# mpriessner/MultiModalSpectralTransformer

Measured on NVIDIA B200. Metric: generated SMILES tokens/sec, higher is better.
Workload: dtype bf16

## Files before the change

### multimodalspectraltransformer_b200/csrc/engine.cu

```cuda
#include "engine.cuh"
#include "kernels_simt.cuh"
#include "kernels_tc.cuh"
#include "kernels_decode.cuh"
#include "kernels_ffn.cuh"
#include "kernels_attn5.cuh"
#include "kernels_compact.cuh"
#include "kernels_beam.cuh"
#include "kernels_smiles.cuh"

#include <algorithm>
#include <cstdlib>
#include <cstring>

namespace mmt {
thread_local std::string g_last_error;

static const char* kEmbedKeys[5] = {
    "linear_spec_embedding_1H.point_embedding_layer_1H.fc_H",
    "linear_spec_embedding_13C.point_embedding_layer_13C.fc_C",
    "linear_spec_embedding_HSQC.point_embedding_layer_HSQC.fc_HSQC",
    "linear_spec_embedding_COSY.point_embedding_layer_COSY.fc_COSY",
    "linear_spec_embedding_IR.linear_spec_embedding_IR"};
static const char* kEncNames[6] = {"encoder_1H", "encoder_13C", "encoder_HSQC", "encoder_COSY", "encoder_IR", "encoder_cross"};

static void prof_pre(mmt_engine* e, cudaStream_t s) {
    if (!e->profiling) return;
    cudaEvent_t a, b;
    cudaEventCreate(&a); cudaEventCreate(&b);
    cudaEventRecord(a, s);
    e->prof_open = {a, b};
}
static int check_launch(mmt_engine* e, const char* what, cudaStream_t s = nullptr, double work = 0.0) {
    e->launches++;
    cudaError_t err = cudaGetLastError();
    if (e->profiling && e->prof_open.first) {
        cudaEventRecord(e->prof_open.second, s);
        e->prof_records.push_back({what, e->prof_open.first, e->prof_open.second, work});
        e->prof_open = {nullptr, nullptr};
// ... 98 lines not shown
}

static int launch_ln(mmt_engine* e, LnParams& p, int ngroups, int maxM, cudaStream_t s) {
    if (maxM <= 0) return 0;
    dim3 grid((maxM + 7) / 8, ngroups);
    prof_pre(e, s);
    bias_res_layernorm<<<grid, 256, 0, s>>>(p);
    return check_launch(e, "bias_res_layernorm", s);
}

typedef CUresult (*PFN_tmapEncodeTiled)(CUtensorMap*, CUtensorMapDataType, cuuint32_t, void*, const cuuint64_t*, const cuuint64_t*,
                                        const cuuint32_t*, const cuuint32_t*, CUtensorMapInterleave, CUtensorMapSwizzle,
                                        CUtensorMapL2promotion, CUtensorMapFloatOOBfill);
static PFN_tmapEncodeTiled g_encode_tiled = nullptr;

static int tc_init(mmt_engine* e) {
    if (e->tc_ready) return 0;
    if (!g_encode_tiled) {
        void* fn = nullptr;
        cudaDriverEntryPointQueryResult qres;
        MMT_CUDA(cudaGetDriverEntryPoint("cuTensorMapEncodeTiled", &fn, cudaEnableDefault, &qres));
        if (!fn || qres != cudaDriverEntryPointSuccess) MMT_FAIL("cuTensorMapEncodeTiled not available from the driver");
        g_encode_tiled = (PFN_tmapEncodeTiled)fn;
    }
    const int max_smem = TC_MAX_STAGES * TC_STAGE_BYTES_WSPLIT + 1024;
    MMT_CUDA(cudaFuncSetAttribute(gemm_bf16_tc<TC_EPI_STORE>, cudaFuncAttributeMaxDynamicSharedMemorySize, max_smem));
    MMT_CUDA(cudaFuncSetAttribute(gemm_bf16_tc<TC_EPI_LN>, cudaFuncAttributeMaxDynamicSharedMemorySize, max_smem));
    MMT_CUDA(cudaFuncSetAttribute(attn_encoder_tc5, cudaFuncAttributeMaxDynamicSharedMemorySize, A5_SMEM_BYTES));
    MMT_CUDA(cudaFuncSetAttribute(ffn_fused_tc<TC_EPI_STORE, 1>, cudaFuncAttributeMaxDynamicSharedMemorySize, ff_smem_bytes<1>()));
    MMT_CUDA(cudaFuncSetAttribute(ffn_fused_tc<TC_EPI_LN, 1>, cudaFuncAttributeMaxDynamicSharedMemorySize, ff_smem_bytes<1>()));
    MMT_CUDA(cudaFuncSetAttribute(ffn_fused_tc<TC_EPI_STORE, 0>, cudaFuncAttributeMaxDynamicSharedMemorySize, ff_smem_bytes<0>()));
    MMT_CUDA(cudaFuncSetAttribute(ffn_fused_tc<TC_EPI_LN, 0>, cudaFuncAttributeMaxDynamicSharedMemorySize, ff_smem_bytes<0>()));
    MMT_CUDA(cudaFuncSetAttribute(ffn_fused_tc<TC_EPI_LN, 0, 1>, cudaFuncAttributeMaxDynamicSharedMemorySize, ff_smem_bytes<0, 1>()));
    e->tc_ready = true;
    return 0;
}

static int make_tmap(CUtensorMap* m, const __nv_bfloat16* ptr, int64_t rows, int64_t cols, int64_t ld, int box_rows = TC_BM) {
    if (((uintptr_t)ptr & 15) || (ld * 2) % 16) MMT_FAIL("tensor map: operand must be 16-byte aligned with a 16-byte multiple row pitch");
    cuuint64_t dims[2] = {(cuuint64_t)cols, (cuuint64_t)rows};
    cuuint64_t strides[1] = {(cuuint64_t)ld * 2};
    cuuint32_t box[2] = {(cuuint32_t)TC_BK, (cuuint32_t)box_rows};
    cuuint32_t estr[2] = {1, 1};
    CUresult r = g_encode_tiled(m, CU_TENSOR_MAP_DATA_TYPE_BFLOAT16, 2, (void*)ptr, dims, strides, box, estr, CU_TENSOR_MAP_INTERLEAVE_NONE,
                                CU_TENSOR_MAP_SWIZZLE_128B, CU_TENSOR_MAP_L2_PROMOTION_L2_256B, CU_TENSOR_MAP_FLOAT_OOB_FILL_NONE);
    if (r != CUDA_SUCCESS) MMT_FAIL("cuTensorMapEncodeTiled failed with CUresult " + std::to_string((int)r));
    return 0;
}

static TcGemmParams tc_params(int M, int N, int K) {
    TcGemmParams p;
    memset(&p, 0, sizeof(p));
    p.M = M; p.N = N; p.K = K; p.splits = 1; p.eps = 1e-5f;
    p.S_in = M > 0 ? M : 1; p.stride_b = 0; p.stride_s = 1; p.off = 0;
    return p;
}

static int sample_init(mmt_engine* e) {
    if (e->sample_ready) return 0;
    MMT_CUDA(cudaFuncSetAttribute(sample_tokens, cudaFuncAttributeMaxDynamicSharedMemorySize, (int)sample_smem_bytes(VOCAB_MAX)));
    e->sample_ready = true;
    return 0;
}

struct TcChain { const __nv_bfloat16 *W, *Wlo; const float* bias; float* out; int64_t ld; };
static int launch_tc(mmt_engine* e, TcGemmParams& p, const __nv_bfloat16* A, int64_t lda, const __nv_bfloat16* W, int epi, cudaStream_t s,
// ... 757 lines not shown
        p.bias = w.in_b; p.out_f32 = b.qkv; p.ld_f32 = e->use_kv_epilogue ? D : 3 * D;
        p.kv_append = e->use_kv_epilogue ? (e->kv_tok_major && H % 8 == 0 ? 2 : 1) : 0; p.kv_pool = reinterpret_cast<__nv_bfloat16*>(pool); p.block_table = b.block_table; p.pps = pps; p.step = step; p.kv_heads = H;
        MMT_TRY(launch_tc(e, p, b.x16, D, e->Wb(w.in_w), TC_EPI_STORE, s, e->dec_proj_single ? nullptr : e->Wlo(w.in_w), pdl_u));
    } else {
        GemmParams p = gemm_params(3 * D, D, 3 * D, 0);
        p.g[0].A = b.x; p.g[0].lda = D; p.g[0].W = w.in_w; p.g[0].bias = w.in_b; p.g[0].C = b.qkv; p.g[0].M = M;
        p.splits = 1; p.part_stride = Nw * D;
        MMT_TRY(launch_gemm(e, p, 1, M, s));
    }
    prof_pre(e, s);
    const unsigned sa_blocks = (unsigned)((Nw * (H / 4) + 7) / 8);
    if (bf16 && e->use_kv_epilogue && e->kv_tok_major && H % 8 == 0)
        launch_args(decode_self_attention_tm<8>, dim3((unsigned)((Nw * (H / 8) + 7) / 8)), dim3(256), 0, s, pdl_u, (const float*)b.qkv, (const __nv_bfloat16*)reinterpret_cast<__nv_bfloat16*>(pool), (const int*)b.block_table, pps, Nw, H, scale, step, b.att16);
    else if (bf16 && e->use_kv_epilogue) launch_args(decode_self_attention_g8<8, __nv_bfloat16, false>, dim3(sa_blocks), dim3(256), 0, s, pdl_u, (const float*)b.qkv, reinterpret_cast<__nv_bfloat16*>(pool), (const int*)b.block_table, pps, Nw, H, scale, step, (float*)nullptr, b.att16);
    else if (bf16) launch_args(decode_self_attention_g8<8, __nv_bfloat16>, dim3(sa_blocks), dim3(256), 0, s, pdl_u, (const float*)b.qkv, reinterpret_cast<__nv_bfloat16*>(pool), (const int*)b.block_table, pps, Nw, H, scale, step, (float*)nullptr, b.att16);
    else decode_self_attention_g8<8, float><<<sa_blocks, 256, 0, s>>>(b.qkv, reinterpret_cast<float*>(pool), b.block_table, pps, Nw, H, scale, step, b.att, b.att16);
    return check_launch(e, "decode_self_attention", s);
}

static int decode_cross_attention_layer(mmt_engine* e, const mmt_decode_args& a, const DecBuffers& b, const char* ckv, int64_t Nw, int Bmw,
                                        bool bf16, bool pdl_u, cudaStream_t s) {
    const int H = e->desc.n_heads, dh = D / H;
    const float scale = 1.0f / sqrtf((float)dh);
    if (dh != 8) MMT_FAIL("decoder head dim must be 8");
    const unsigned attn_blocks = (unsigned)((Nw * H + 7) / 8);
    prof_pre(e, s);
    if (bf16 && a.n_cand >= 8 && e->use_tc_attention)
        launch_args(decode_cross_attention_tc, dim3(H, Bmw), dim3(256), dx_smem_bytes(a.S), s, pdl_u, (const float*)b.qc, reinterpret_cast<const __nv_bfloat16*>(ckv), (int64_t)a.S, (const int*)b.nk, (const int*)b.row_start, (const float*)b.kbias_c, (int)a.n_cand, H, scale, (float*)nullptr, b.att16);
    else if (bf16) launch_args(decode_cross_attention<8, __nv_bfloat16>, dim3(attn_blocks), dim3(256), 0, s, pdl_u, (const float*)b.qc, reinterpret_cast<const __nv_bfloat16*>(ckv), (int64_t)a.S, (const int*)b.nk, (const int*)b.row_start, (const float*)b.kbias_c, (int)a.n_cand, Nw, H, scale, (float*)nullptr, b.att16);
    else decode_cross_attention<8, float><<<attn_blocks, 256, 0, s>>>(b.qc, reinterpret_cast<const float*>(ckv), a.S, b.nk, b.row_start, b.kbias_c, a.n_cand, Nw, H, scale, b.att, b.att16);
    return check_launch(e, "decode_cross_attention", s);
}

struct DecOps {
    mmt_engine* e; const DecBuffers& b; int64_t Nw; bool pdl_u; cudaStream_t s;
    int ln(const float* part, int splits, const float* bias, const float* gamma, const float* beta) const {
        LnParams q;
        memset(&q, 0, sizeof(q));
        q.splits = splits; q.part_stride = Nw * D; q.eps = 1e-5f;
        LnGroup& g = q.g[0];
        g.part = part; g.bias = bias; g.res = b.x; g.gamma = gamma; g.beta = beta; g.out = b.x; g.out_bf16 = b.x16; g.M = (int)Nw;
        g.S_in = (int)Nw; g.stride_b = 0; g.stride_s = 1; g.off = 0;
        return launch_ln(e, q, 1, (int)Nw, s);
    }
    int gemm(const float* A, int64_t lda, const float* W, const float* bias, float* C, int N, int K, int act, int splits) const {
        GemmParams p = gemm_params(N, K, N, act);
        p.g[0].A = A; p.g[0].lda = lda; p.g[0].W = W; p.g[0].bias = bias; p.g[0].C = C; p.g[0].M = (int)Nw;
        p.splits = splits; p.part_stride = Nw * D;
        return launch_gemm(e, p, 1, (int)Nw, s);
    }
    const __nv_bfloat16* plo(const float* w) const { return e->dec_proj_single ? nullptr : e->Wlo(w); }
    const __nv_bfloat16* dlo(const float* w) const { return e->dec_ffn_single ? nullptr : e->Wlo(w); }
    int tc(const __nv_bfloat16* A, int64_t lda, const float* W, const float* bias, float* C32, __nv_bfloat16* C16, int N, int K, int act, int splits) const {
        TcGemmParams p = tc_params((int)Nw, N, K);
        p.bias = bias; p.act = act; p.out_f32 = C32; p.ld_f32 = N; p.out_b16 = C16; p.ld_b16 = N;
        p.splits = splits; p.part_stride = Nw * D;
        return launch_tc(e, p, A, lda, e->Wb(W), TC_EPI_STORE, s, plo(W), pdl_u);
    }
    int tc_ln(const __nv_bfloat16* A, int64_t lda, const float* W, const float* bias, int K, const float* gamma, const float* beta,
              const TcChain* chain = nullptr) const {
        TcGemmParams p = tc_params((int)Nw, D, K);
        p.bias = bias; p.res = b.x; p.gamma = gamma; p.beta = beta;
        p.out_f32 = b.x; p.ld_f32 = D; p.out_b16 = b.x16; p.ld_b16 = D;
        return launch_tc(e, p, A, lda, e->Wb(W), TC_EPI_LN, s, plo(W), pdl_u, chain);
    }
};

static int decode_self_tail_layer(const DecOps& o, const LayerW& w, bool bf16) {
    const DecBuffers& b = o.b;
    if (bf16) {
        if (o.e->use_gemm_chain && o.Nw <= 24576) {
            const TcChain ch{o.e->Wb(w.ca_in_w), o.plo(w.ca_in_w), w.ca_in_b, b.qc, D};
            MMT_TRY(o.tc_ln(b.att16, D, w.out_w, w.out_b, D, w.n1_w, w.n1_b, &ch));
        } else {
            MMT_TRY(o.tc_ln(b.att16, D, w.out_w, w.out_b, D, w.n1_w, w.n1_b));
            MMT_TRY(o.tc(b.x16, D, w.ca_in_w, w.ca_in_b, b.qc, nullptr, D, D, 0, 1));
        }
    } else {
        MMT_TRY(o.gemm(b.att, D, w.out_w, nullptr, b.part, D, D, 0, 1));
        MMT_TRY(o.ln(b.part, 1, w.out_b, w.n1_w, w.n1_b));
        MMT_TRY(o.gemm(b.x, D, w.ca_in_w, w.ca_in_b, b.qc, D, D, 0, 1));
    }
    return 0;
}

static int decode_cross_tail_layer(const DecOps& o, const LayerW& w, int l, bool bf16, float* x2 = nullptr) {
    mmt_engine* e = o.e;
    const DecBuffers& b = o.b;
    const int M = (int)o.Nw, F = e->desc.d_ff;
    cudaStream_t s = o.s;
    auto keep_x2 = [&]() -> int {
        if (x2) MMT_CUDA(cudaMemcpyAsync(x2, b.x, (size_t)M * D * sizeof(float), cudaMemcpyDeviceToDevice, s));
        return 0;
    };
    if (bf16) {
        const bool ffn_pro = e->use_ffn_prologue && M >= 2048;
        if (!ffn_pro) { MMT_TRY(o.tc_ln(b.att16, D, w.ca_out_w, w.ca_out_b, D, w.n2_w, w.n2_b)); MMT_TRY(keep_x2()); }
        if (M >= 2048) {
            FfnParams f = ffn_params(M, F);
            f.b1 = w.l1_b; f.bias = w.l2_b; f.res = b.x; f.gamma = w.n3_w; f.beta = w.n3_b; f.out_f32 = b.x; f.out_b16 = b.x16;
            if (getenv("MMT_FFN_DEBUG")) {
                if (!e->ffn_dbg) { MMT_CUDA(cudaMallocManaged(&e->ffn_dbg, 4096 * 16 * sizeof(long long))); memset(e->ffn_dbg, 0, 4096 * 16 * sizeof(long long)); }
// ... 77 lines not shown
            if (cl_ffn) {
                MMT_TRY(tc_init(e));
                MMT_TRY(make_tmap(&q.tmW1, e->Wb(w.l1_w), d.d_ff, D, D));
                MMT_TRY(make_tmap(&q.tmW2, e->Wb(w.l2_w), D, d.d_ff, d.d_ff));
                q.b1 = w.l1_b; q.b2 = w.l2_b; q.n3_w = w.n3_w; q.n3_b = w.n3_b; q.x_out = b.x;
            }
            q.in_w = w.in_w; q.in_b = w.in_b; q.out_w = w.out_w; q.out_b = w.out_b; q.n1_w = w.n1_w; q.n1_b = w.n1_b;
            q.kv_pool = b.kv_pool + (size_t)l * b.pool_pages * 2 * PAGE_TOKENS * D * b.kv_esz; q.block_table = b.block_table; q.pps = pps;
            q.step = step;
            q.in_w16 = e->Wb(w.in_w); q.out_w16 = e->Wb(w.out_w); q.cq_w16 = e->Wb(w.ca_in_w); q.co_w16 = e->Wb(w.ca_out_w);
            q.cq_w = w.ca_in_w; q.cq_b = w.ca_in_b; q.co_w = w.ca_out_w; q.co_b = w.ca_out_b; q.n2_w = w.n2_w; q.n2_b = w.n2_b;
            q.ckv = b.cross_kv + (size_t)l * 2 * R * D * b.kv_esz; q.rows_total = a.S;
            q.nk = b.nk; q.row_start = b.row_start; q.kbias_c = b.kbias_c; q.n_cand = a.n_cand;
            q.x2 = b.x; q.x2_16 = bf16 ? b.x16 : nullptr; q.M = Nw; q.scale = scale; q.eps = 1e-5f;
            q.dbg = (e->da_dbg && l == 3) ? e->da_dbg : nullptr;
            prof_pre(e, s);
            const bool pdl_l = pdl && !(l == 0 && r.serial_first);
            if (cl_ffn) launch_kernel_cluster(decode_attn<8, __nv_bfloat16, true>, dim3(blocks), dim3(DA_THREADS), DA_SMEM_BYTES_CL, s, pdl_l, DA_CL, q);
            else if (bf16) launch_kernel(decode_attn<8, __nv_bfloat16>, dim3(blocks), dim3(DA_THREADS), DA_SMEM_BYTES, s, pdl_l, q);
            else launch_kernel(decode_attn<8, float>, dim3(blocks), dim3(DA_THREADS), DA_SMEM_BYTES, s, pdl_l, q);
            MMT_TRY(check_launch(e, "decode_attn", s));
            if (cl_ffn) continue;
            if (bf16) {
                FfnParams f = ffn_params(M, d.d_ff);
                f.b1 = w.l1_b; f.splits = ffn_splits; f.out_f32 = b.part; f.part_stride = Nw * D;
                f.dbg = (e->da_dbg && l == 3) ? e->da_dbg + 2048 * 16 : nullptr;
                MMT_TRY(launch_ffn(e, f, b.x16, D, e->Wb(w.l1_w), o.dlo(w.l1_w), e->Wb(w.l2_w), o.dlo(w.l2_w), TC_EPI_STORE, s, pdl));
            } else {
                MMT_TRY(o.gemm(b.x, D, w.l1_w, w.l1_b, b.h, d.d_ff, D, 1, 1));
                MMT_TRY(o.gemm(b.h, d.d_ff, w.l2_w, nullptr, b.part, D, d.d_ff, 0, ffn_splits));
            }
        }
    } else {
        prof_pre(e, s);
        if (r.trg) launch_args(decode_embed, dim3((unsigned)((Nw + 3) / 4)), dim3(128), 0, s, pdl_u, r.trg + n0, 0, 3, Nw, ldn, e->W("embed_trg.weight"), e->W("pe_trg.weight"), (int)d.vocab, step, b.x, b.x16);
        else launch_args(decode_embed, dim3((unsigned)((Nw + 3) / 4)), dim3(128), 0, s, pdl_u, (const int64_t*)(r.tokens + n0), 1, 3, Nw, ldn, e->W("embed_trg.weight"), e->W("pe_trg.weight"), (int)d.vocab, step, b.x, b.x16);
        MMT_TRY(check_launch(e, "decode_embed", s));

        for (int l = 0; l < d.n_dec_layers; ++l) {
            const LayerW& w = e->dec[l];
            char* pool = b.kv_pool + (size_t)l * b.pool_pages * 2 * PAGE_TOKENS * D * b.kv_esz;
            const char* ckv = b.cross_kv + (size_t)l * 2 * R * D * b.kv_esz;
            MMT_TRY(decode_self_attention_layer(e, w, b, pool, pps, Nw, bf16, pdl_u, s));
            MMT_TRY(decode_self_tail_layer(o, w, bf16));
            MMT_TRY(decode_cross_attention_layer(e, a, b, ckv, Nw, Bmw, bf16, pdl_u, s));
            MMT_TRY(decode_cross_tail_layer(o, w, l, bf16));
        }
    }
    SampleParams sp;
    memset(&sp, 0, sizeof(sp));
    sp.x = b.x; sp.W = e->W("fc_out.weight"); sp.b = e->W("fc_out.bias"); sp.V = d.vocab; sp.N = Nw; sp.ldn = ldn;
    sp.temperature = a.temperature; sp.mode = r.mode;
    int smc = a.rng_sm_count > 0 ? a.rng_sm_count : e->sm_count;
    int mts = a.rng_max_threads_per_sm > 0 ? a.rng_max_threads_per_sm : e->max_threads_per_sm;
    int64_t Nrng = r.per_memory_rng ? a.n_cand : (a.N_total > 0 ? a.N_total : N_total);
    sp.rng.seed = a.philox_seed; sp.rng.offset = a.philox_offset; sp.rng.numel = Nrng * d.vocab;
    sp.rng.threads = torch_rng_threads(sp.rng.numel, smc, mts);
    sp.rng_inc = torch_rng_increment(sp.rng.numel, smc, mts);
    sp.rng_dev = b.rng_state;
    sp.seq_index_base = a.seq_index_base + n0;
    if (r.per_memory_rng) { sp.rng_cand = a.n_cand; sp.rng_col_steps = a.max_len; }
    sp.tokens = r.tokens ? r.tokens + n0 : nullptr; sp.probs = r.probs ? r.probs + n0 : nullptr;
    sp.logits = r.logits ? r.logits + n0 * d.vocab : nullptr;
    sp.target = r.target ? r.target + n0 : nullptr; sp.target_prob = r.target_prob ? r.target_prob + n0 : nullptr;
    sp.ctl.step = b.ctl; sp.ctl.done_ctas = b.ctl + 1; sp.ctl.nonpad = (r.mode == 0) ? b.ctl + 8 : nullptr;
    sp.advance = 1;
    if (fused && ffn_splits > 0) {
        const LayerW& pw = e->dec[d.n_dec_layers - 1];
        sp.part = b.part; sp.splits = ffn_splits; sp.part_stride = Nw * D;
        sp.pbias = pw.l2_b; sp.pgamma = pw.n3_w; sp.pbeta = pw.n3_b; sp.eps = 1e-5f;
    }
    prof_pre(e, s);
    {
        sp.rows_per_warp = Nw >= 8192 ? SAMPLE_NR : 1;
        const int rpc = sp.part ? 2 : 8 * sp.rows_per_warp;
        const int64_t groups = (Nw + rpc - 1) / rpc;
        MMT_TRY(sample_init(e));
        launch_kernel(sample_tokens, dim3((unsigned)std::min<int64_t>(groups, (int64_t)e->sm_count * 4)), dim3(256), sample_smem_bytes(sp.V), s, pdl || pdl_u, sp);
// ... 346 lines not shown
}
int64_t mmt_weight_total(const mmt_model_desc* desc) { if (check_desc(desc)) return -1; return build_registry(*desc).total; }

int32_t mmt_create(const mmt_model_desc* desc, const float* h_weights, int64_t n_floats, int32_t device, mmt_engine** out) {
    if (!out) MMT_FAIL("null out");
    *out = nullptr;
    MMT_TRY(check_desc(desc));
    int ndev = 0;
    if (cudaGetDeviceCount(&ndev) != cudaSuccess || ndev == 0) MMT_FAIL("no CUDA device: this engine has no CPU fallback");
    if (device < 0 || device >= ndev) MMT_FAIL("bad device index");
    cudaDeviceProp prop;
    MMT_CUDA(cudaGetDeviceProperties(&prop, device));
    if (prop.major != 10) MMT_FAIL(std::string("device is sm_") + std::to_string(prop.major * 10 + prop.minor) + "; this library is built for sm_100a (B200) only");
    MMT_CUDA(cudaSetDevice(device));
    mmt_engine* e = new mmt_engine();
    e->desc = *desc; e->device = device; e->sm_count = prop.multiProcessorCount; e->max_threads_per_sm = prop.maxThreadsPerMultiProcessor; e->total_mem = prop.totalGlobalMem;
    e->reg = build_registry(*desc);
    if (getenv("MMT_NO_GRAPH")) e->use_graph = false;
    if (getenv("MMT_NO_PDL")) e->use_pdl = false;
    if (getenv("MMT_NO_GRAPH_CACHE")) e->use_graph_cache = false;
    if (const char* v = getenv("MMT_GRAPH_STEPS")) e->graph_steps = std::max(1, atoi(v));
    if (getenv("MMT_NO_ENC_STREAMS")) e->use_enc_streams = false;
    if (const char* v = getenv("MMT_DECODE_LANES")) e->decode_lanes = std::max(1, atoi(v));
    if (getenv("MMT_DENSE_ENCODER")) e->use_compact = false;
    if (getenv("MMT_NO_TC_ATTENTION")) e->use_tc_attention = false;
    if (getenv("MMT_TC5_ATTENTION")) e->use_tc5_attention = true;
    if (const char* v = getenv("MMT_FFN_SPLITS")) { int k = atoi(v); if (k == 1 || k == 2 || k == 4 || k == 8 || k == 16 || k == 32) e->ffn_splits_override = k; }
    if (getenv("MMT_TC_ATTENTION_FP32")) e->tc_attention_fp32 = true;
    if (const char* v = getenv("MMT_FUSED_DECODE_ROWS")) e->fused_decode_rows = atoi(v);
    if (getenv("MMT_DEC_FFN_TWO_TERM")) e->dec_ffn_single = false;
    if (getenv("MMT_DEC_PROJ_TWO_TERM")) e->dec_proj_single = false;
    if (const char* v = getenv("MMT_PDL_ROWS")) e->pdl_rows = atoi(v);
    if (getenv("MMT_NO_GEMM_CHAIN")) e->use_gemm_chain = false;
    if (getenv("MMT_NO_FFN_WIDE")) e->use_ffn_wide = false;
    if (getenv("MMT_NO_KV_EPILOGUE")) e->use_kv_epilogue = false;
    if (getenv("MMT_KV_HEAD_MAJOR")) e->kv_tok_major = false;
    if (getenv("MMT_CLUSTER_FFN")) e->use_cluster_ffn = true;
    if (getenv("MMT_NO_FFN_PROLOGUE")) e->use_ffn_prologue = false;
    if (getenv("MMT_ENC_FFN_SINGLE")) e->enc_ffn_single = true;
    if (const char* v = getenv("MMT_DECODE_LANES_LARGE")) e->decode_lanes_large = std::max(1, atoi(v));
    if (const char* v = getenv("MMT_MAX_WAVE_SEQS")) e->max_wave_seqs = std::max(1, atoi(v));
    if (n_floats != e->reg.total) { delete e; MMT_FAIL("weight blob has " + std::to_string(n_floats) + " floats, expected " + std::to_string(build_registry(*desc).total)); }
    auto fail = [&](const std::string& m) { mmt_destroy(e); g_last_error = m; return 1; };
    if (cudaMalloc(&e->w32, n_floats * sizeof(float)) != cudaSuccess) return fail("cudaMalloc weights failed");
    if (cudaMalloc(&e->w16, n_floats * sizeof(__nv_bfloat16)) != cudaSuccess) return fail("cudaMalloc bf16 weights failed");
    if (cudaMemcpy(e->w32, h_weights, n_floats * sizeof(float), cudaMemcpyHostToDevice) != cudaSuccess) return fail("weight H2D copy failed");
    if (cudaMalloc(&e->w16lo, n_floats * sizeof(__nv_bfloat16)) != cudaSuccess) return fail("cudaMalloc bf16 weights (low term) failed");
    f32_to_bf16_split<<<(unsigned)((n_floats + 255) / 256), 256>>>(e->w32, n_floats, e->w16, e->w16lo);
    if (cudaDeviceSynchronize() != cudaSuccess) return fail(std::string("bf16 weight conversion failed: ") + cudaGetErrorString(cudaGetLastError()));
    if (cudaMallocHost(&e->h_pinned, 1024 * sizeof(int32_t)) != cudaSuccess) return fail("cudaMallocHost failed");
    for (int k = 0; k < 6; ++k) {
        e->enc[k].resize(desc->n_enc_layers);
        for (int l = 0; l < desc->n_enc_layers; ++l) fill_layer(e, e->enc[k][l], std::string(kEncNames[k]) + ".layers." + std::to_string(l), false);
    }
    e->dec.resize(desc->n_dec_layers);
    for (int l = 0; l < desc->n_dec_layers; ++l) fill_layer(e, e->dec[l], "decoder.layers." + std::to_string(l), true);
    *out = e;
    return 0;
}

void mmt_destroy(mmt_engine* e) {
    if (!e) return;
    cudaSetDevice(e->device);
    cudaDeviceSynchronize();
    if (e->w32) cudaFree(e->w32);
    if (e->w16) cudaFree(e->w16);
// ... 659 lines not shown
```

### multimodalspectraltransformer_b200/csrc/engine.cuh

```cuda
#pragma once
#include <mutex>
#include <string>
#include <unordered_map>
#include <vector>

#include "../../include/mmt_b200.h"
#include "common.cuh"

namespace mmt {

extern thread_local std::string g_last_error;

#define MMT_FAIL(msg)                                                                   \
    do {                                                                                \
        ::mmt::g_last_error = std::string(__FILE__) + ":" + std::to_string(__LINE__) + ": " + (msg); \
        return 1;                                                                       \
    } while (0)
#define MMT_CUDA(call)                                                                  \
    do {                                                                                \
        cudaError_t err__ = (call);                                                     \
        if (err__ != cudaSuccess) MMT_FAIL(std::string(#call) + " -> " + cudaGetErrorString(err__)); \
    } while (0)
#define MMT_TRY(call)                                                                   \
    do {                                                                                \
// ... 67 lines not shown
    T* get(size_t n) {
        size_t bytes = (n * sizeof(T) + 255) & ~size_t(255);
        T* p = plan ? nullptr : reinterpret_cast<T*>(base + off);
        off += bytes;
        return p;
    }
};

}

struct mmt_engine {
    mmt_model_desc desc;
    int device = 0, sm_count = 0, max_threads_per_sm = 0;
    size_t total_mem = 0;
    mmt::Registry reg;
    float* w32 = nullptr;
    __nv_bfloat16* w16 = nullptr;
    __nv_bfloat16* w16lo = nullptr;
    std::vector<mmt::LayerW> enc[6];
    std::vector<mmt::LayerW> dec;
    char* arena = nullptr;
    size_t arena_bytes = 0;
    int64_t launches = 0;
    bool use_graph = true;
    int fused_decode_rows = 2048;
    int max_wave_seqs = 0;
    bool enc_ffn_single = false;
    bool use_ffn_prologue = true;
    bool use_cluster_ffn = false;
    bool kv_tok_major = true;
    bool use_kv_epilogue = true;
    bool use_ffn_wide = true;
    bool use_gemm_chain = true;
    bool dec_proj_single = true;
    bool sample_ready = false;
    bool dec_ffn_single = true;
    bool use_compact = true;
    struct GraphEntry { std::vector<uint64_t> key; cudaGraphExec_t exec; int64_t launches_per_group; uint64_t stamp; };
    std::vector<GraphEntry> graph_cache;
    uint64_t graph_cache_clock = 0;
    bool use_graph_cache = true;
    bool use_tc_attention = true;
    bool use_tc5_attention = false;
    bool tc_attention_fp32 = false;
    int ffn_splits_override = 0;
    bool use_enc_streams = true;
    cudaStream_t enc_stream[5] = {nullptr, nullptr, nullptr, nullptr, nullptr};
    cudaEvent_t enc_ev[6] = {nullptr, nullptr, nullptr, nullptr, nullptr, nullptr};
    int graph_steps = 16;
    int pdl_rows = 4096;
    bool use_pdl = true;
    cudaStream_t cap_stream[4] = {nullptr, nullptr, nullptr, nullptr};
    cudaEvent_t lane_ev[4] = {nullptr, nullptr, nullptr, nullptr};
    int decode_lanes = 2;
    int decode_lanes_large = 1;
    long long* ffn_dbg = nullptr;
    long long* da_dbg = nullptr;
    bool da_ready = false;
    bool tc_ready = false;
    cudaEvent_t poll_ev[2] = {nullptr, nullptr};
    int32_t* h_pinned = nullptr;
    struct ProfRecord { const char* name; cudaEvent_t a, b; double work; };
    bool profiling = false;
    std::pair<cudaEvent_t, cudaEvent_t> prof_open{nullptr, nullptr};
    std::vector<ProfRecord> prof_records;

// ... 10 lines not shown
```

### multimodalspectraltransformer_b200/csrc/kernels_simt.cuh

```cuda
#pragma once
#include "common.cuh"
#include "philox.cuh"

namespace mmt {

constexpr int GEMM_MAX_GROUPS = 6;

struct GemmGroup {
    const float* A;
    const int64_t* a_row_off;
    const float* W;
    const float* bias;
    float* C;
    const int* M_dev;
    int64_t lda;
    int M;
};

enum { GEMM_OUT_ROWMAJOR = 0, GEMM_OUT_HEADMAJOR = 1 };

struct GemmParams {
    GemmGroup g[GEMM_MAX_GROUPS];
    int N, K;
    int splits;
// ... 1084 lines not shown
        if (s > m) {
            float corr = expf(m - s);
            l *= corr;
#pragma unroll
            for (int d = 0; d < DH; ++d) acc[d] *= corr;
            m = s;
        }
        float e = expf(s - m);
        l += e;
        float v[DH];
        KV::unpack(rv, v);
#pragma unroll
        for (int d = 0; d < DH; ++d) acc[d] = fmaf(e, v[d], acc[d]);
    }
    float M = warp_max(m);
    float corr = (m == MMT_NEG_INF) ? 0.f : expf(m - M);
    l = warp_sum(l * corr);
#pragma unroll
    for (int d = 0; d < DH; ++d) acc[d] = warp_sum(acc[d] * corr);
    if (lane < DH) {
        float v = 0.f;
#pragma unroll
        for (int d = 0; d < DH; ++d) if (lane == d) v = acc[d];
        if (out) out[n * D + h * DH + lane] = v / l;
        if (out16) out16[n * D + h * DH + lane] = __float2bfloat16_rn(v / l);
    }
}

__host__ __device__ inline int dx_keys_padded(int nk) { return (nk + 31) / 32 * 32; }
__host__ __device__ inline size_t dx_smem_bytes(int key_bound) {
    const int nkp = dx_keys_padded(key_bound);
    return (size_t)nkp * 8 * 2 + (size_t)8 * (nkp + 8) * 2 + (size_t)nkp * 4;
}
__global__ void __launch_bounds__(256) decode_cross_attention_tc(const float* q_in, const __nv_bfloat16* kv, int64_t rows_total,
                                                                 const int* nk, const int* row_start, const float* kbias_c,
                                                                 int n_cand, int H, float scale, float* out, __nv_bfloat16* out16) {
    extern __shared__ __align__(16) unsigned char dx_smem[];
    constexpr int DH = 8;
    constexpr float LOG2E = 1.4426950408889634f;
    pdl_launch_dependents();
    const int h = blockIdx.x;
    const int64_t b = blockIdx.y;
    const int cnt = nk[b];
    const int64_t r0 = row_start[b];
    const int nkp_max = dx_keys_padded((int)rows_total), nkp = dx_keys_padded(cnt);
    const int vstride = nkp_max + 8;
    __nv_bfloat16* Ks = reinterpret_cast<__nv_bfloat16*>(dx_smem);
    __nv_bfloat16* Vt = Ks + (size_t)nkp_max * DH;
    float* bs = reinterpret_cast<float*>(Vt + (size_t)DH * vstride);
    const __nv_bfloat16* Kh = kv + (((int64_t)b * 2 + 0) * H + h) * rows_total * DH;
    const __nv_bfloat16* Vh = kv + (((int64_t)b * 2 + 1) * H + h) * rows_total * DH;
    for (int j = threadIdx.x; j < nkp; j += blockDim.x) {
        uint4 k = make_uint4(0u, 0u, 0u, 0u), v = k;
        float bias = MMT_NEG_INF;
        if (j < cnt) {
            k = *reinterpret_cast<const uint4*>(Kh + (int64_t)j * DH);
            v = *reinterpret_cast<const uint4*>(Vh + (int64_t)j * DH);
            bias = kbias_c[r0 + j] * LOG2E;
        }
        *reinterpret_cast<uint4*>(Ks + (size_t)j * DH) = k;
        const uint32_t vw[4] = {v.x, v.y, v.z, v.w};
#pragma unroll
        for (int c = 0; c < 4; ++c) {
            Vt[(2 * c) * vstride + j] = __ushort_as_bfloat16((unsigned short)(vw[c] & 0xffffu));
            Vt[(2 * c + 1) * vstride + j] = __ushort_as_bfloat16((unsigned short)(vw[c] >> 16));
        }
        bs[j] = bias;
    }
    __syncthreads();
    pdl_wait();
    const int warp = threadIdx.x >> 5, lane = threadIdx.x & 31, nwarps = blockDim.x >> 5;
    const int gq = lane >> 2, tq = lane & 3;
    const float qscale = scale * LOG2E;
    for (int tile = warp; tile * 16 < n_cand; tile += nwarps) {
        const int c_lo = tile * 16 + gq, c_hi = c_lo + 8;
        const int64_t n_lo = b * n_cand + c_lo, n_hi = b * n_cand + c_hi;
        uint32_t qh[2], ql[2];
        {
            float2 a = make_float2(0.f, 0.f), c = a;
            if (c_lo < n_cand) a = *reinterpret_cast<const float2*>(q_in + n_lo * D + h * DH + 2 * tq);
            if (c_hi < n_cand) c = *reinterpret_cast<const float2*>(q_in + n_hi * D + h * DH + 2 * tq);
            split_pair(a.x * qscale, a.y * qscale, qh[0], ql[0]);
            split_pair(c.x * qscale, c.y * qscale, qh[1], ql[1]);
        }
        const uint32_t qa[4] = {qh[0], qh[1], ql[0], ql[1]};
        float acc[4] = {0.f, 0.f, 0.f, 0.f};
        float m_lo = MMT_NEG_INF, m_hi = MMT_NEG_INF, l_lo = 0.f, l_hi = 0.f;
        for (int kb = 0; kb < nkp; kb += 32) {
            float sc[4][4];
#pragma unroll
            for (int nt = 0; nt < 4; ++nt) {
                const float2 bb = *reinterpret_cast<const float2*>(bs + kb + nt * 8 + 2 * tq);
                sc[nt][0] = bb.x; sc[nt][1] = bb.y; sc[nt][2] = bb.x; sc[nt][3] = bb.y;
                const uint32_t kf = *reinterpret_cast<const uint32_t*>(Ks + (size_t)(kb + nt * 8 + gq) * DH + 2 * tq);
                mma_bf16_16816(sc[nt], qa, kf, kf);
            }
            float bm_lo = fmaxf(fmaxf(fmaxf(sc[0][0], sc[0][1]), fmaxf(sc[1][0], sc[1][1])), fmaxf(fmaxf(sc[2][0], sc[2][1]), fmaxf(sc[3][0], sc[3][1])));
            float bm_hi = fmaxf(fmaxf(fmaxf(sc[0][2], sc[0][3]), fmaxf(sc[1][2], sc[1][3])), fmaxf(fmaxf(sc[2][2], sc[2][3]), fmaxf(sc[3][2], sc[3][3])));
            bm_lo = fmaxf(bm_lo, __shfl_xor_sync(0xffffffffu, bm_lo, 1)); bm_lo = fmaxf(bm_lo, __shfl_xor_sync(0xffffffffu, bm_lo, 2));
            bm_hi = fmaxf(bm_hi, __shfl_xor_sync(0xffffffffu, bm_hi, 1)); bm_hi = fmaxf(bm_hi, __shfl_xor_sync(0xffffffffu, bm_hi, 2));
            const float nm_lo = fmaxf(m_lo, bm_lo), nm_hi = fmaxf(m_hi, bm_hi);
            if (__any_sync(0xffffffffu, nm_lo != m_lo || nm_hi != m_hi)) {
                const float corr_lo = ex2_approx(m_lo - nm_lo), corr_hi = ex2_approx(m_hi - nm_hi);
                m_lo = nm_lo; m_hi = nm_hi;
                l_lo *= corr_lo; l_hi *= corr_hi;
                acc[0] *= corr_lo; acc[1] *= corr_lo; acc[2] *= corr_hi; acc[3] *= corr_hi;
            }
#pragma unroll
            for (int half = 0; half < 2; ++half) {
                uint32_t ph[4];
#pragma unroll
                for (int nt = 0; nt < 2; ++nt) {
                    const float* c = sc[half * 2 + nt];
                    const float e0 = ex2_approx(c[0] - m_lo), e1 = ex2_approx(c[1] - m_lo);
                    const float e2 = ex2_approx(c[2] - m_hi), e3 = ex2_approx(c[3] - m_hi);
                    l_lo += e0 + e1; l_hi += e2 + e3;
                    const __nv_bfloat162 p01 = __floats2bfloat162_rn(e0, e1), p23 = __floats2bfloat162_rn(e2, e3);
                    ph[nt * 2] = *reinterpret_cast<const uint32_t*>(&p01);
                    ph[nt * 2 + 1] = *reinterpret_cast<const uint32_t*>(&p23);
                }
                const uint32_t* vr = reinterpret_cast<const uint32_t*>(Vt + (size_t)gq * vstride + kb + half * 16 + 2 * tq);
                mma_bf16_16816(acc, ph, vr[0], vr[4]);
            }
        }
        l_lo += __shfl_xor_sync(0xffffffffu, l_lo, 1); l_lo += __shfl_xor_sync(0xffffffffu, l_lo, 2);
        l_hi += __shfl_xor_sync(0xffffffffu, l_hi, 1); l_hi += __shfl_xor_sync(0xffffffffu, l_hi, 2);
        const int col = h * DH + 2 * tq;
        if (c_lo < n_cand) {
            const float o0 = acc[0] / l_lo, o1 = acc[1] / l_lo;
            if (out) *reinterpret_cast<float2*>(out + n_lo * D + col) = make_float2(o0, o1);
            if (out16) *reinterpret_cast<__nv_bfloat162*>(out16 + n_lo * D + col) = __floats2bfloat162_rn(o0, o1);
        }
        if (c_hi < n_cand) {
            const float o0 = acc[2] / l_hi, o1 = acc[3] / l_hi;
            if (out) *reinterpret_cast<float2*>(out + n_hi * D + col) = make_float2(o0, o1);
            if (out16) *reinterpret_cast<__nv_bfloat162*>(out16 + n_hi * D + col) = __floats2bfloat162_rn(o0, o1);
        }
    }
}

struct SampleParams {
    const float* x;
    const float* W;
    const float* b;
    int V;
    int64_t N;
    int64_t ldn;
    float temperature;
    int mode;
    RngGeom rng;
    uint64_t rng_inc;
    const uint64_t* rng_dev;
    int64_t seq_index_base;
    int64_t rng_cand;
    int64_t rng_col_steps;
    int64_t* tokens;
    float* probs;
    float* logits;
    const int64_t* target;
// ... 310 lines not shown
```

Measured before the change: 17.31 million.

## Fuse decoder cross-attention Q projection with attention in one tcgen05 kernel

Adds a decode_cross_fused kernel that computes the cross-attention Q projection on tensor memory via UMMA and runs the per-head attention over the memory in the same block. Per-head K/V planes are streamed through a shared-memory ring with bulk async copies and mbarriers. The self-attention tail now stops after the output projection and LN, so the separate Q GEMM, its global round-trip and one launch disappear. The shared attention loop is factored into dx_attend_rounds with a V fragment loader, and the fused path loads V with ldmatrix.trans. This costs a large shared-memory footprint and a TMEM allocation per block, which may limit occupancy.

```diff
diff --git a/multimodalspectraltransformer_b200/csrc/engine.cu b/multimodalspectraltransformer_b200/csrc/engine.cu
--- a/multimodalspectraltransformer_b200/csrc/engine.cu
+++ b/multimodalspectraltransformer_b200/csrc/engine.cu
@@ -4,6 +4,7 @@
 #include "kernels_decode.cuh"
 #include "kernels_ffn.cuh"
 #include "kernels_attn5.cuh"
+#include "kernels_cross.cuh"
 #include "kernels_compact.cuh"
 #include "kernels_beam.cuh"
 #include "kernels_smiles.cuh"
@@ -168,6 +169,7 @@
     MMT_CUDA(cudaFuncSetAttribute(ffn_fused_tc<TC_EPI_STORE, 0>, cudaFuncAttributeMaxDynamicSharedMemorySize, ff_smem_bytes<0>()));
     MMT_CUDA(cudaFuncSetAttribute(ffn_fused_tc<TC_EPI_LN, 0>, cudaFuncAttributeMaxDynamicSharedMemorySize, ff_smem_bytes<0>()));
     MMT_CUDA(cudaFuncSetAttribute(ffn_fused_tc<TC_EPI_LN, 0, 1>, cudaFuncAttributeMaxDynamicSharedMemorySize, ff_smem_bytes<0, 1>()));
+    MMT_CUDA(cudaFuncSetAttribute(decode_cross_fused, cudaFuncAttributeMaxDynamicSharedMemorySize, XF_MAX_SMEM));
     e->tc_ready = true;
     return 0;
 }
@@ -991,6 +993,33 @@
     return check_launch(e, "decode_cross_attention", s);
 }
 
+static bool cross_fused(const mmt_engine* e, const mmt_decode_args& a, bool bf16) {
+    return bf16 && a.n_cand >= 8 && e->use_tc_attention && e->use_cross_fused;
+}
+static int decode_cross_fused_layer(mmt_engine* e, const mmt_decode_args& a, const DecBuffers& b, const LayerW& w, const __nv_bfloat16* wlo,
+                                    const char* ckv, int64_t Nw, int Bmw, bool pdl_u, cudaStream_t s) {
+    const int H = e->desc.n_heads;
+    if (D / H != 8 || H > XF_MAX_SLOTS) MMT_FAIL("decode_cross_fused: decoder heads must be of dim 8");
+    MMT_TRY(tc_init(e));
+    CrossFusedParams p;
+    memset(&p, 0, sizeof(p));
+    MMT_TRY(make_tmap(&p.tmX, b.x16, Nw, D, D));
+    MMT_TRY(make_tmap(&p.tmW, e->Wb(w.ca_in_w), D, D, D));
+    p.wsplit = wlo != nullptr;
+    if (wlo) MMT_TRY(make_tmap(&p.tmW2, wlo, D, D, D));
+    p.bias = w.ca_in_b;
+    p.kv = reinterpret_cast<const __nv_bfloat16*>(ckv); p.rows_total = a.S;
+    p.nk = b.nk; p.row_start = b.row_start; p.kbias_c = b.kbias_c;
+    p.n_cand = a.n_cand; p.H = H; p.scale = 1.0f / sqrtf((float)(D / H));
+    p.ring_bytes = XF_MIN_SLOTS * xf_slot_bytes(a.S);
+    p.out16 = b.att16;
+    const size_t smem = xf_smem_bytes(a.S, p.wsplit);
+    if (smem > XF_MAX_SMEM) MMT_FAIL("decode_cross_fused: memory of " + std::to_string(a.S) + " rows exceeds shared memory");
+    prof_pre(e, s);
+    launch_kernel(decode_cross_fused, dim3((unsigned)((a.n_cand + XF_ROWS - 1) / XF_ROWS), (unsigned)Bmw), dim3(XF_THREADS), smem, s, pdl_u, p);
+    return check_launch(e, "decode_cross_fused", s, 2.0 * Nw * D * D * (p.wsplit ? 2 : 1));
+}
+
 struct DecOps {
     mmt_engine* e; const DecBuffers& b; int64_t Nw; bool pdl_u; cudaStream_t s;
     int ln(const float* part, int splits, const float* bias, const float* gamma, const float* beta) const {
@@ -1025,8 +1054,9 @@
     }
 };
 
-static int decode_self_tail_layer(const DecOps& o, const LayerW& w, bool bf16) {
+static int decode_self_tail_layer(const DecOps& o, const LayerW& w, bool bf16, bool qc = true) {
     const DecBuffers& b = o.b;
+    if (bf16 && !qc) return o.tc_ln(b.att16, D, w.out_w, w.out_b, D, w.n1_w, w.n1_b);
     if (bf16) {
         if (o.e->use_gemm_chain && o.Nw <= 24576) {
             const TcChain ch{o.e->Wb(w.ca_in_w), o.plo(w.ca_in_w), w.ca_in_b, b.qc, D};
@@ -1170,6 +1200,7 @@
             }
         }
     } else {
+        const bool xf = cross_fused(e, a, bf16);
         prof_pre(e, s);
         if (r.trg) launch_args(decode_embed, dim3((unsigned)((Nw + 3) / 4)), dim3(128), 0, s, pdl_u, r.trg + n0, 0, 3, Nw, ldn, e->W("embed_trg.weight"), e->W("pe_trg.weight"), (int)d.vocab, step, b.x, b.x16);
         else launch_args(decode_embed, dim3((unsigned)((Nw + 3) / 4)), dim3(128), 0, s, pdl_u, (const int64_t*)(r.tokens + n0), 1, 3, Nw, ldn, e->W("embed_trg.weight"), e->W("pe_trg.weight"), (int)d.vocab, step, b.x, b.x16);
@@ -1180,8 +1211,9 @@
             char* pool = b.kv_pool + (size_t)l * b.pool_pages * 2 * PAGE_TOKENS * D * b.kv_esz;
             const char* ckv = b.cross_kv + (size_t)l * 2 * R * D * b.kv_esz;
             MMT_TRY(decode_self_attention_layer(e, w, b, pool, pps, Nw, bf16, pdl_u, s));
-            MMT_TRY(decode_self_tail_layer(o, w, bf16));
-            MMT_TRY(decode_cross_attention_layer(e, a, b, ckv, Nw, Bmw, bf16, pdl_u, s));
+            MMT_TRY(decode_self_tail_layer(o, w, bf16, !xf));
+            if (xf) MMT_TRY(decode_cross_fused_layer(e, a, b, w, o.plo(w.ca_in_w), ckv, Nw, Bmw, pdl_u, s));
+            else MMT_TRY(decode_cross_attention_layer(e, a, b, ckv, Nw, Bmw, bf16, pdl_u, s));
             MMT_TRY(decode_cross_tail_layer(o, w, l, bf16));
         }
     }
@@ -1594,6 +1626,7 @@
     if (getenv("MMT_DEC_PROJ_TWO_TERM")) e->dec_proj_single = false;
     if (const char* v = getenv("MMT_PDL_ROWS")) e->pdl_rows = atoi(v);
     if (getenv("MMT_NO_GEMM_CHAIN")) e->use_gemm_chain = false;
+    if (getenv("MMT_NO_CROSS_FUSED")) e->use_cross_fused = false;
     if (getenv("MMT_NO_FFN_WIDE")) e->use_ffn_wide = false;
     if (getenv("MMT_NO_KV_EPILOGUE")) e->use_kv_epilogue = false;
     if (getenv("MMT_KV_HEAD_MAJOR")) e->kv_tok_major = false;
diff --git a/multimodalspectraltransformer_b200/csrc/engine.cuh b/multimodalspectraltransformer_b200/csrc/engine.cuh
--- a/multimodalspectraltransformer_b200/csrc/engine.cuh
+++ b/multimodalspectraltransformer_b200/csrc/engine.cuh
@@ -123,6 +123,7 @@
     bool use_kv_epilogue = true;
     bool use_ffn_wide = true;
     bool use_gemm_chain = true;
+    bool use_cross_fused = true;
     bool dec_proj_single = true;
     bool sample_ready = false;
     bool dec_ffn_single = true;
diff --git a/multimodalspectraltransformer_b200/csrc/kernels_cross.cuh b/multimodalspectraltransformer_b200/csrc/kernels_cross.cuh
--- /dev/null
+++ b/multimodalspectraltransformer_b200/csrc/kernels_cross.cuh
@@ -0,0 +1,191 @@
+#pragma once
+#include "kernels_simt.cuh"
+#include "kernels_tc.cuh"
+
+namespace mmt {
+
+constexpr int XF_THREADS = 512;
+constexpr int XF_ROWS = 128;
+constexpr int XF_MAX_SLOTS = 16;
+constexpr int XF_MIN_SLOTS = 2;
+constexpr int XF_MAX_SMEM = 226 * 1024;
+
+struct CrossFusedParams {
+    CUtensorMap tmX;
+    CUtensorMap tmW, tmW2;
+    int wsplit;
+    const float* bias;
+    const __nv_bfloat16* kv;
+    int64_t rows_total;
+    const int* nk; const int* row_start; const float* kbias_c;
+    int n_cand, H;
+    float scale;
+    int ring_bytes;
+    __nv_bfloat16* out16;
+};
+
+__host__ __device__ inline int xf_slot_bytes(int nk) { return dx_keys_padded(nk) * 8 * 2 * 2; }
+__host__ __device__ inline int xf_op_bytes(int wsplit) { return (wsplit ? 6 : 4) * TC_SLAB_BYTES; }
+__host__ inline size_t xf_smem_bytes(int key_bound, int wsplit) {
+    return 1024 + (size_t)xf_op_bytes(wsplit) + (size_t)XF_MIN_SLOTS * xf_slot_bytes(key_bound) + (size_t)dx_keys_padded(key_bound) * 4;
+}
+
+__device__ __forceinline__ void bulk_load(void* smem_dst, const void* src, uint32_t bytes, uint64_t* bar) {
+    asm volatile("cp.async.bulk.shared::cluster.global.mbarrier::complete_tx::bytes [%0], [%1], %2, [%3];"
+                 ::"r"(smem_u32(smem_dst)), "l"(reinterpret_cast<uint64_t>(src)), "r"(bytes), "r"(smem_u32(bar)) : "memory");
+}
+
+__device__ __forceinline__ int xf_q_word(int row, int pair) { return row * 64 + (pair ^ ((row & 7) << 2)); }
+
+__global__ void __launch_bounds__(XF_THREADS, 2) decode_cross_fused(const __grid_constant__ CrossFusedParams p) {
+    extern __shared__ uint8_t smem_raw[];
+    __shared__ __align__(8) uint64_t op_bar, acc_bar;
+    __shared__ __align__(8) uint64_t full_bar[XF_MAX_SLOTS], empty_bar[XF_MAX_SLOTS];
+    __shared__ uint32_t tmem_slot;
+    constexpr int DH = 8;
+    constexpr float LOG2E = 1.4426950408889634f;
+
+    uint8_t* smem = smem_raw + ((1024u - (smem_u32(smem_raw) & 1023u)) & 1023u);
+    uint8_t* ring = smem + xf_op_bytes(p.wsplit);
+    const int warp = threadIdx.x >> 5, lane = threadIdx.x & 31;
+    const int64_t b = blockIdx.y;
+    const int c0 = blockIdx.x * XF_ROWS;
+    const int rows = min(XF_ROWS, p.n_cand - c0);
+    const int64_t row0 = b * p.n_cand + c0;
+    const int cnt = p.nk[b];
+    const int64_t r0 = p.row_start[b];
+    const int nkp = dx_keys_padded(cnt);
+    const int slot_bytes = xf_slot_bytes(cnt);
+    const int ns = max(1, min(p.H, p.ring_bytes / max(slot_bytes, 1)));
+    float* bs = reinterpret_cast<float*>(ring + p.ring_bytes);
+    const __nv_bfloat16* kvb = p.kv + (b * 2 * p.H) * p.rows_total * DH;
+    const int64_t plane = p.rows_total * DH;
+
+    pdl_launch_dependents();
+    if (threadIdx.x == 0) {
+        tma_prefetch_desc(&p.tmX);
+        tma_prefetch_desc(&p.tmW);
+        if (p.wsplit) tma_prefetch_desc(&p.tmW2);
+        mbar_init(&op_bar, 1);
+        mbar_init(&acc_bar, 1);
+        for (int s = 0; s < ns; ++s) { mbar_init(&full_bar[s], 1); mbar_init(&empty_bar[s], XF_THREADS / 64); }
+        fence_barrier_init();
+    }
+    if (warp == 0) tmem_alloc(&tmem_slot, XF_ROWS);
+    for (int i = threadIdx.x; i < ns * 2 * (nkp - cnt); i += XF_THREADS) {
+        const int s = i / (2 * (nkp - cnt)), rr = i % (2 * (nkp - cnt));
+        const int kvsel = rr / (nkp - cnt), j = cnt + rr % (nkp - cnt);
+        *reinterpret_cast<uint4*>(ring + (size_t)s * slot_bytes + ((size_t)kvsel * nkp + j) * DH * 2) = make_uint4(0u, 0u, 0u, 0u);
+    }
+    for (int j = threadIdx.x; j < nkp; j += XF_THREADS) bs[j] = j < cnt ? p.kbias_c[r0 + j] * LOG2E : MMT_NEG_INF;
+    tc_fence_before();
+    __syncthreads();
+    tc_fence_after();
+    const uint32_t tmem_base = tmem_slot;
+
+    auto issue_head = [&](int h, int s) {
+        uint8_t* dst = ring + (size_t)s * slot_bytes;
+        const uint32_t bytes = (uint32_t)cnt * DH * 2;
+        mbar_arrive_expect_tx(&full_bar[s], 2 * bytes);
+        if (bytes) {
+            bulk_load(dst, kvb + (int64_t)h * plane, bytes, &full_bar[s]);
+            bulk_load(dst + (size_t)nkp * DH * 2, kvb + (int64_t)(p.H + h) * plane, bytes, &full_bar[s]);
+        }
+    };
+    if (threadIdx.x == 0) {
+        mbar_arrive_expect_tx(&op_bar, (uint32_t)xf_op_bytes(p.wsplit));
+        for (int ks = 0; ks < 2; ++ks) {
+            tma_load_2d(smem + (2 + ks) * TC_SLAB_BYTES, &p.tmW, &op_bar, ks * TC_BK, 0);
+            if (p.wsplit) tma_load_2d(smem + (4 + ks) * TC_SLAB_BYTES, &p.tmW2, &op_bar, ks * TC_BK, 0);
+        }
+        for (int s = 0; s < ns; ++s) issue_head(s, s);
+        pdl_wait();
+        for (int ks = 0; ks < 2; ++ks) tma_load_2d(smem + ks * TC_SLAB_BYTES, &p.tmX, &op_bar, ks * TC_BK, (int)row0);
+        mbar_wait(&op_bar, 0);
+        tc_fence_after();
+        constexpr uint32_t idesc = umma_idesc_bf16(TC_BM, TC_BN);
+        for (int ks = 0; ks < 2; ++ks) {
+            const uint64_t adesc = umma_desc_sw128(smem_u32(smem + ks * TC_SLAB_BYTES));
+            const uint64_t bdesc = umma_desc_sw128(smem_u32(smem + (2 + ks) * TC_SLAB_BYTES));
+#pragma unroll
+            for (int k = 0; k < TC_BK / 16; ++k)
+                umma_bf16(tmem_base, adesc + (uint64_t)(2 * k), bdesc + (uint64_t)(2 * k), idesc, (ks > 0 || k > 0) ? 1u : 0u);
+            if (p.wsplit) {
+                const uint64_t bdesc2 = umma_desc_sw128(smem_u32(smem + (4 + ks) * TC_SLAB_BYTES));
+#pragma unroll
+                for (int k = 0; k < TC_BK / 16; ++k)
+                    umma_bf16(tmem_base, adesc + (uint64_t)(2 * k), bdesc2 + (uint64_t)(2 * k), idesc, 1u);
+            }
+        }
+        umma_commit(&acc_bar);
+    }
+    pdl_wait();
+    const float qscale = p.scale * LOG2E;
+    uint32_t* Qh = reinterpret_cast<uint32_t*>(smem);
+    uint32_t* Ql = Qh + XF_ROWS * 64;
+    {
+        const int q = warp & 3;
+        const int r = q * 32 + lane;
+        mbar_wait(&acc_bar, 0);
+        tc_fence_after();
+        {
+            const int col0 = (warp >> 2) * 32;
+            uint32_t a[32];
+            tmem_ld_32x32(tmem_base + ((uint32_t)(q * 32) << 16) + (uint32_t)col0, a);
+            tmem_ld_wait();
+#pragma unroll
+            for (int j = 0; j < 16; j += 4) {
+                uint32_t hi[4], lo[4];
+#pragma unroll
+                for (int u = 0; u < 4; ++u) {
+                    const int c = col0 + 2 * (j + u);
+                    const float2 bb = *reinterpret_cast<const float2*>(p.bias + c);
+                    const float x = __uint_as_float(a[2 * (j + u)]) + bb.x, y = __uint_as_float(a[2 * (j + u) + 1]) + bb.y;
+                    split_pair(x * qscale, y * qscale, hi[u], lo[u]);
+                    if (r >= rows) { hi[u] = 0u; lo[u] = 0u; }
+                }
+                const int w = xf_q_word(r, col0 / 2 + j);
+                *reinterpret_cast<uint4*>(Qh + w) = make_uint4(hi[0], hi[1], hi[2], hi[3]);
+                *reinterpret_cast<uint4*>(Ql + w) = make_uint4(lo[0], lo[1], lo[2], lo[3]);
+            }
+        }
+    }
+    tc_fence_before();
+    __syncthreads();
+    if (warp == 0) { tc_fence_after(); tmem_dealloc(tmem_base, XF_ROWS); }
+
+    const int gq = lane >> 2, tq = lane & 3;
+    const int wt = warp & 7, hg = warp >> 3;
+    const int rl = wt * 16 + gq, rh = rl + 8;
+    const bool active = wt * 16 < rows;
+    for (int h = hg; h < p.H; h += 2) {
+        const int s = h % ns;
+        const uint32_t use = (uint32_t)(h / ns) & 1u;
+        mbar_wait(&full_bar[s], use);
+        if (active) {
+            const uint8_t* slot = ring + (size_t)s * slot_bytes;
+            const __nv_bfloat16* Ks = reinterpret_cast<const __nv_bfloat16*>(slot);
+            const uint32_t vaddr = smem_u32(slot + (size_t)nkp * DH * 2) + (uint32_t)lane * DH * 2;
+            const int pr = h * 4 + tq;
+            const uint32_t qa[4] = {Qh[xf_q_word(rl, pr)], Qh[xf_q_word(rh, pr)], Ql[xf_q_word(rl, pr)], Ql[xf_q_word(rh, pr)]};
+            float acc[4];
+            float l_lo, l_hi;
+            dx_attend_rounds(qa, Ks, bs, nkp, gq, tq,
+                             [&](int kb, uint32_t (&v)[4]) { ldmatrix_x4_trans(v, vaddr + (uint32_t)kb * DH * 2); }, acc, l_lo, l_hi);
+            const int col = h * DH + 2 * tq;
+            if (rl < rows) *reinterpret_cast<__nv_bfloat162*>(p.out16 + (row0 + rl) * D + col) = __floats2bfloat162_rn(acc[0] / l_lo, acc[1] / l_lo);
+            if (rh < rows) *reinterpret_cast<__nv_bfloat162*>(p.out16 + (row0 + rh) * D + col) = __floats2bfloat162_rn(acc[2] / l_hi, acc[3] / l_hi);
+        }
+        __syncwarp();
+        if (h + ns < p.H) {
+            if (lane == 0) mbar_arrive(&empty_bar[s]);
+            if (warp == hg * 8 && lane == 0) {
+                mbar_wait(&empty_bar[s], use);
+                issue_head(h + ns, s);
+            }
+            __syncwarp();
+        }
+    }
+}
+
+}
diff --git a/multimodalspectraltransformer_b200/csrc/kernels_simt.cuh b/multimodalspectraltransformer_b200/csrc/kernels_simt.cuh
--- a/multimodalspectraltransformer_b200/csrc/kernels_simt.cuh
+++ b/multimodalspectraltransformer_b200/csrc/kernels_simt.cuh
@@ -1140,6 +1140,54 @@
     const int nkp = dx_keys_padded(key_bound);
     return (size_t)nkp * 8 * 2 + (size_t)8 * (nkp + 8) * 2 + (size_t)nkp * 4;
 }
+template <class VFrag>
+__device__ __forceinline__ void dx_attend_rounds(const uint32_t (&qa)[4], const __nv_bfloat16* Ks, const float* bs, int nkp, int gq, int tq,
+                                                 VFrag vfrag, float (&acc)[4], float& l_lo, float& l_hi) {
+    constexpr int DH = 8;
+    acc[0] = acc[1] = acc[2] = acc[3] = 0.f;
+    float m_lo = MMT_NEG_INF, m_hi = MMT_NEG_INF;
+    l_lo = 0.f; l_hi = 0.f;
+    for (int kb = 0; kb < nkp; kb += 32) {
+        float sc[4][4];
+        uint32_t vf[4];
+        vfrag(kb, vf);
+#pragma unroll
+        for (int nt = 0; nt < 4; ++nt) {
+            const float2 bb = *reinterpret_cast<const float2*>(bs + kb + nt * 8 + 2 * tq);
+            sc[nt][0] = bb.x; sc[nt][1] = bb.y; sc[nt][2] = bb.x; sc[nt][3] = bb.y;
+            const uint32_t kf = *reinterpret_cast<const uint32_t*>(Ks + (size_t)(kb + nt * 8 + gq) * DH + 2 * tq);
+            mma_bf16_16816(sc[nt], qa, kf, kf);
+        }
+        float bm_lo = fmaxf(fmaxf(fmaxf(sc[0][0], sc[0][1]), fmaxf(sc[1][0], sc[1][1])), fmaxf(fmaxf(sc[2][0], sc[2][1]), fmaxf(sc[3][0], sc[3][1])));
+        float bm_hi = fmaxf(fmaxf(fmaxf(sc[0][2], sc[0][3]), fmaxf(sc[1][2], sc[1][3])), fmaxf(fmaxf(sc[2][2], sc[2][3]), fmaxf(sc[3][2], sc[3][3])));
+        bm_lo = fmaxf(bm_lo, __shfl_xor_sync(0xffffffffu, bm_lo, 1)); bm_lo = fmaxf(bm_lo, __shfl_xor_sync(0xffffffffu, bm_lo, 2));
+        bm_hi = fmaxf(bm_hi, __shfl_xor_sync(0xffffffffu, bm_hi, 1)); bm_hi = fmaxf(bm_hi, __shfl_xor_sync(0xffffffffu, bm_hi, 2));
+        const float nm_lo = fmaxf(m_lo, bm_lo), nm_hi = fmaxf(m_hi, bm_hi);
+        if (__any_sync(0xffffffffu, nm_lo != m_lo || nm_hi != m_hi)) {
+            const float corr_lo = ex2_approx(m_lo - nm_lo), corr_hi = ex2_approx(m_hi - nm_hi);
+            m_lo = nm_lo; m_hi = nm_hi;
+            l_lo *= corr_lo; l_hi *= corr_hi;
+            acc[0] *= corr_lo; acc[1] *= corr_lo; acc[2] *= corr_hi; acc[3] *= corr_hi;
+        }
+#pragma unroll
+        for (int half = 0; half < 2; ++half) {
+            uint32_t ph[4];
+#pragma unroll
+            for (int nt = 0; nt < 2; ++nt) {
+                const float* c = sc[half * 2 + nt];
+                const float e0 = ex2_approx(c[0] - m_lo), e1 = ex2_approx(c[1] - m_lo);
+                const float e2 = ex2_approx(c[2] - m_hi), e3 = ex2_approx(c[3] - m_hi);
+                l_lo += e0 + e1; l_hi += e2 + e3;
+                const __nv_bfloat162 p01 = __floats2bfloat162_rn(e0, e1), p23 = __floats2bfloat162_rn(e2, e3);
+                ph[nt * 2] = *reinterpret_cast<const uint32_t*>(&p01);
+                ph[nt * 2 + 1] = *reinterpret_cast<const uint32_t*>(&p23);
+            }
+            mma_bf16_16816(acc, ph, vf[2 * half], vf[2 * half + 1]);
+        }
+    }
+    l_lo += __shfl_xor_sync(0xffffffffu, l_lo, 1); l_lo += __shfl_xor_sync(0xffffffffu, l_lo, 2);
+    l_hi += __shfl_xor_sync(0xffffffffu, l_hi, 1); l_hi += __shfl_xor_sync(0xffffffffu, l_hi, 2);
+}
 __global__ void __launch_bounds__(256) decode_cross_attention_tc(const float* q_in, const __nv_bfloat16* kv, int64_t rows_total,
                                                                  const int* nk, const int* row_start, const float* kbias_c,
                                                                  int n_cand, int H, float scale, float* out, __nv_bfloat16* out16) {
@@ -1192,47 +1240,13 @@
             split_pair(c.x * qscale, c.y * qscale, qh[1], ql[1]);
         }
         const uint32_t qa[4] = {qh[0], qh[1], ql[0], ql[1]};
-        float acc[4] = {0.f, 0.f, 0.f, 0.f};
-        float m_lo = MMT_NEG_INF, m_hi = MMT_NEG_INF, l_lo = 0.f, l_hi = 0.f;
-        for (int kb = 0; kb < nkp; kb += 32) {
-            float sc[4][4];
-#pragma unroll
-            for (int nt = 0; nt < 4; ++nt) {
-                const float2 bb = *reinterpret_cast<const float2*>(bs + kb + nt * 8 + 2 * tq);
-                sc[nt][0] = bb.x; sc[nt][1] = bb.y; sc[nt][2] = bb.x; sc[nt][3] = bb.y;
-                const uint32_t kf = *reinterpret_cast<const uint32_t*>(Ks + (size_t)(kb + nt * 8 + gq) * DH + 2 * tq);
-                mma_bf16_16816(sc[nt], qa, kf, kf);
-            }
-            float bm_lo = fmaxf(fmaxf(fmaxf(sc[0][0], sc[0][1]), fmaxf(sc[1][0], sc[1][1])), fmaxf(fmaxf(sc[2][0], sc[2][1]), fmaxf(sc[3][0], sc[3][1])));
-            float bm_hi = fmaxf(fmaxf(fmaxf(sc[0][2], sc[0][3]), fmaxf(sc[1][2], sc[1][3])), fmaxf(fmaxf(sc[2][2], sc[2][3]), fmaxf(sc[3][2], sc[3][3])));
-            bm_lo = fmaxf(bm_lo, __shfl_xor_sync(0xffffffffu, bm_lo, 1)); bm_lo = fmaxf(bm_lo, __shfl_xor_sync(0xffffffffu, bm_lo, 2));
-            bm_hi = fmaxf(bm_hi, __shfl_xor_sync(0xffffffffu, bm_hi, 1)); bm_hi = fmaxf(bm_hi, __shfl_xor_sync(0xffffffffu, bm_hi, 2));
-            const float nm_lo = fmaxf(m_lo, bm_lo), nm_hi = fmaxf(m_hi, bm_hi);
-            if (__any_sync(0xffffffffu, nm_lo != m_lo || nm_hi != m_hi)) {
-                const float corr_lo = ex2_approx(m_lo - nm_lo), corr_hi = ex2_approx(m_hi - nm_hi);
-                m_lo = nm_lo; m_hi = nm_hi;
-                l_lo *= corr_lo; l_hi *= corr_hi;
-                acc[0] *= corr_lo; acc[1] *= corr_lo; acc[2] *= corr_hi; acc[3] *= corr_hi;
-            }
-#pragma unroll
-            for (int half = 0; half < 2; ++half) {
-                uint32_t ph[4];
-#pragma unroll
-                for (int nt = 0; nt < 2; ++nt) {
-                    const float* c = sc[half * 2 + nt];
-                    const float e0 = ex2_approx(c[0] - m_lo), e1 = ex2_approx(c[1] - m_lo);
-                    const float e2 = ex2_approx(c[2] - m_hi), e3 = ex2_approx(c[3] - m_hi);
-                    l_lo += e0 + e1; l_hi += e2 + e3;
-                    const __nv_bfloat162 p01 = __floats2bfloat162_rn(e0, e1), p23 = __floats2bfloat162_rn(e2, e3);
-                    ph[nt * 2] = *reinterpret_cast<const uint32_t*>(&p01);
-                    ph[nt * 2 + 1] = *reinterpret_cast<const uint32_t*>(&p23);
-                }
-                const uint32_t* vr = reinterpret_cast<const uint32_t*>(Vt + (size_t)gq * vstride + kb + half * 16 + 2 * tq);
-                mma_bf16_16816(acc, ph, vr[0], vr[4]);
-            }
-        }
-        l_lo += __shfl_xor_sync(0xffffffffu, l_lo, 1); l_lo += __shfl_xor_sync(0xffffffffu, l_lo, 2);
-        l_hi += __shfl_xor_sync(0xffffffffu, l_hi, 1); l_hi += __shfl_xor_sync(0xffffffffu, l_hi, 2);
+        float acc[4], l_lo, l_hi;
+        const __nv_bfloat16* vq = Vt + (size_t)gq * vstride + 2 * tq;
+        dx_attend_rounds(qa, Ks, bs, nkp, gq, tq, [&](int kb, uint32_t (&v)[4]) {
+            const uint32_t* v0 = reinterpret_cast<const uint32_t*>(vq + kb);
+            const uint32_t* v1 = reinterpret_cast<const uint32_t*>(vq + kb + 16);
+            v[0] = v0[0]; v[1] = v0[4]; v[2] = v1[0]; v[3] = v1[4];
+        }, acc, l_lo, l_hi);
         const int col = h * DH + 2 * tq;
         if (c_lo < n_cand) {
             const float o0 = acc[0] / l_lo, o1 = acc[1] / l_lo;
```

New measurement: 17.53 million (median of 6 runs). +1.3%, better.
